# HKPolyU-UAV/FLVIS

Measured on AMD Instinct MI355X. Metric: frames/sec/node (640×480 stereo+IMU) + ATE vs CPU ref, EuRoC MH_05, higher is better.
Workload: dtype u8/f32 LK+GFTT, f64 geometry+BA

## Files before the change

### flvis_amd/csrc/dev_geom.hpp

```cpp
#pragma once
#include "dev_math.hpp"

namespace flvis {

FD void project_point(const float* p3, const M3& R, V3 t, const double* K, const double* D, float* out) {
  V3 P{(double)p3[0], (double)p3[1], (double)p3[2]};
  V3 X = R * P + t;
  double z = X.z ? 1. / X.z : 1;
  double x = X.x * z, y = X.y * z;
  double r2 = x * x + y * y, r4 = r2 * r2;
  double a1 = 2 * x * y, a2 = r2 + 2 * x * x, a3 = r2 + 2 * y * y;
  double cdist = 1 + D[0] * r2 + D[1] * r4;
  double xd = x * cdist + D[2] * a1 + D[3] * a2;
  double yd = y * cdist + D[2] * a3 + D[3] * a1;
  out[0] = (float)(xd * K[0] + K[2]);
  out[1] = (float)(yd * K[1] + K[3]);
}

FD void undistort_point(const float* src, const double* K, const double* D, const double* R9, const double* P12,
                        float* dst) {
  double x = (src[0] - K[2]) / K[0], y = (src[1] - K[3]) / K[1];
  double x0 = x, y0 = y;
  for (int j = 0; j < 5; j++) {
    double r2 = x * x + y * y;
    double icdist = 1. / (1 + (D[1] * r2 + D[0]) * r2);
    double deltaX = 2 * D[2] * x * y + D[3] * (r2 + 2 * x * x);
    double deltaY = D[2] * (r2 + 2 * y * y) + 2 * D[3] * x * y;
    x = (x0 - deltaX) * icdist;
    y = (y0 - deltaY) * icdist;
  }
  double xx = R9[0] * x + R9[1] * y + R9[2];
  double yy = R9[3] * x + R9[4] * y + R9[5];
  double ww = 1. / (R9[6] * x + R9[7] * y + R9[8]);
  x = xx * ww;
  y = yy * ww;
  dst[0] = (float)(x * P12[0] + P12[2]);
  dst[1] = (float)(y * P12[5] + P12[6]);
}

__device__ inline V3 triangulate_dlt(double u1, double v1, double u2, double v2, const double* P1, const double* P2) {
  double A[4][4], V[4][4];
#pragma unroll
  for (int j = 0; j < 4; j++) {
    A[0][j] = v1 * P1[8 + j] - P1[4 + j];
    A[1][j] = P1[j] - u1 * P1[8 + j];
    A[2][j] = v2 * P2[8 + j] - P2[4 + j];
    A[3][j] = P2[j] - u2 * P2[8 + j];
  }
#pragma unroll
  for (int i = 0; i < 4; i++)
#pragma unroll
    for (int j = 0; j < 4; j++) V[i][j] = (i == j) ? 1.0 : 0.0;
  for (int sweep = 0; sweep < 30; sweep++) {
    int off = 0;
#pragma unroll
    for (int p = 0; p < 3; p++)
#pragma unroll
      for (int q = p + 1; q < 4; q++) {
        double alpha = 0, beta = 0, gamma = 0;
#pragma unroll
        for (int i = 0; i < 4; i++) {
          alpha += A[i][p] * A[i][p];
          beta += A[i][q] * A[i][q];
          gamma += A[i][p] * A[i][q];
        }
        if (gamma * gamma <= 4.930380657631324e-30 * (alpha * beta)) continue;
        off = 1;
        double zeta = (beta - alpha) / (2.0 * gamma);
        double t = (zeta >= 0 ? 1.0 : -1.0) / (fabs(zeta) + sqrt(1.0 + zeta * zeta));
        double c = 1.0 / sqrt(1.0 + t * t), s = c * t;
#pragma unroll
        for (int i = 0; i < 4; i++) {
          double ap = A[i][p], aq = A[i][q];
          A[i][p] = c * ap - s * aq;
          A[i][q] = s * ap + c * aq;
          double vp = V[i][p], vq = V[i][q];
          V[i][p] = c * vp - s * vq;
          V[i][q] = s * vp + c * vq;
        }
      }
    if (!off) break;
  }
  int best = 0;
  double bn = 1.7976931348623157e308;
#pragma unroll
  for (int j = 0; j < 4; j++) {
    double nn = 0;
#pragma unroll
    for (int i = 0; i < 4; i++) nn += A[i][j] * A[i][j];
    if (nn < bn) {
      bn = nn;
      best = j;
    }
  }
  double vx = 0, vy = 0, vz = 0, vw = 1;
#pragma unroll
  for (int j = 0; j < 4; j++)
    if (j == best) {
      vx = V[0][j];
      vy = V[1][j];
      vz = V[2][j];
      vw = V[3][j];
    }
  return V3{vx / vw, vy / vw, vz / vw};
}

__device__ inline V3 triangulate_two_view(double u1, double v1, double u2, double v2, const SE3d& T1, const SE3d& T2,
                                          double fx, double fy, double cx, double cy) {
  double P1[12], P2[12];
  for (int k = 0; k < 2; k++) {
    const SE3d& T = k == 0 ? T1 : T2;
    double* P = k == 0 ? P1 : P2;
    M3 R = q_to_mat(T.q);
    double T34[3][4] = {{R.m[0][0], R.m[0][1], R.m[0][2], T.t.x}, {R.m[1][0], R.m[1][1], R.m[1][2], T.t.y},
                        {R.m[2][0], R.m[2][1], R.m[2][2], T.t.z}};
    for (int j = 0; j < 4; j++) {
      P[j] = fx * T34[0][j] + 0 * T34[1][j] + cx * T34[2][j];
      P[4 + j] = 0 * T34[0][j] + fy * T34[1][j] + cy * T34[2][j];
      P[8 + j] = 0 * T34[0][j] + 0 * T34[1][j] + 1 * T34[2][j];
    }
  }
  return triangulate_dlt(u1, v1, u2, v2, P1, P2);
}

FD float f_error(const double* F, double x1, double y1, double x2, double y2) {
  double a = F[0] * x1 + F[1] * y1 + F[2], b = F[3] * x1 + F[4] * y1 + F[5], c = F[6] * x1 + F[7] * y1 + F[8];
  double s2 = 1. / (a * a + b * b);
  double dd2 = x2 * a + y2 * b + c;
  a = F[0] * x2 + F[3] * y2 + F[6];
  b = F[1] * x2 + F[4] * y2 + F[7];
  c = F[2] * x2 + F[5] * y2 + F[8];
  double s1 = 1. / (a * a + b * b);
  double dd1 = x1 * a + y1 * b + c;
  return (float)fmax(dd1 * dd1 * s1, dd2 * dd2 * s2);
}

FD void proj_edge(const SE3d& T, V3 pw, double zu, double zv, double fx, double fy, double cx, double cy, double* e,
                  double (*J)[6]) {
  V3 X = g2o_map(T, pw);
  double x = X.x, y = X.y, zz = X.z, z2 = zz * zz;
  e[0] = zu - (x / zz * fx + cx);
  e[1] = zv - (y / zz * fy + cy);
  if (J) {
    J[0][0] = x * y / z2 * fx;
    J[0][1] = -(1 + (x * x / z2)) * fx;
    J[0][2] = y / zz * fx;
    J[0][3] = -1. / zz * fx;
    J[0][4] = 0;
    J[0][5] = x / z2 * fx;
    J[1][0] = (1 + y * y / z2) * fy;
    J[1][1] = -x * y / z2 * fy;
    J[1][2] = -x / zz * fy;
    J[1][3] = 0;
    J[1][4] = -1. / zz * fy;
    J[1][5] = y / z2 * fy;
// ... 36 lines not shown
```

### flvis_amd/csrc/frame_schedule.cpp

```cpp
#include <algorithm>
#include <chrono>
#include <cstring>
#include <thread>
#include <vector>

#include "pipeline_host.hpp"

using namespace flvis;

static void fill_pyr(Pipeline* pl, PyrSel& ps, uint8_t* const* l0, uint8_t* const* l1, const int* cur, int flip, int levels) {
  ps.levels = levels;
  for (int l = 0; l <= levels; l++) {
    ps.lvl[l] = ImgSel{{l0[l], l1 ? l1[l] : l0[l]}, cur, flip, nullptr};
    ps.w[l] = pl->lw[l];
    ps.h[l] = pl->lh[l];
    ps.pitch[l] = pl->lpitch[l];
    ps.stride[l] = pl->lstride[l];
    ps.bx[l] = pl->lbx;
    ps.by[l] = pl->lby;
  }
}

unsigned flvis::pyramid_levels(hipStream_t ds, bool bordered, ImgSel src0, int spitch0, size_t sstride0, bool ingest, bool level0_is_buffer,
                               const PyrSel& pyr, int S, const int* active) {
// ... 328 lines not shown
  {
    LaunchJoins j(pl, L, st, p.kj);
    head_signals = !pl->feedback_used && j.fold_signal(J_HEAD);
    head_posts = !idle_step && j.fold_post(J_IMG);
    if (head_prepare) launch_frame_head_prepare(st, p, L->d_time, L->d_progress, frame_no);
    else launch_frame_head(st, p, L->d_time, L->d_progress, frame_no);
  }
  if (pl->feedback_used) launch_apply_correction(st, p);
  pe(0, st);
  if (!head_signals) join_signal(pl, L, J_HEAD, st);
}

void Frame::local_map_tail(hipEvent_t* p18, bool timed) {
  if (with_local_map && (pl->frames_fed % pl->ba_every) == 0) {
    if (L->ba_pending) launch_local_map(pl, L, J_FE, true, nullptr);
    if (pl->defer_ba) L->ba_pending = true;
    else if (L->endf_valid) launch_local_map(pl, L, J_ENDF, false, p18);
    else launch_local_map(pl, L, J_FE, true, p18);
  } else if (!with_local_map) {
    if (cmd_pending) {
      if (L->ba_launches > 0) join_wait(pl, L, st, J_BA(L->ba_launches - 1));
      launch_kfq_drop(st, p);
    } else hipMemcpyAsync(p.kfq_head, p.kfq_tail, sizeof(unsigned) * S, hipMemcpyDeviceToDevice, st);
    if (timed) {
      pb(18, st);
      pe(18, st);
      L->prof18_rec[(size_t)pl->prof_step] = 1;
    }
  }
}

void Frame::frame_end(bool backpressure, bool with_innovate) {
  LaunchJoins j(pl, L, st, p.kj);
  if (with_innovate) j.wait(J_TRI);
  if (backpressure) lane_backpressure_wait(pl, L, &j, 0, with_innovate ? 1 : pl->nba_lane);
  pb(with_innovate ? 16 : 17, st);
  L->endf_valid = j.fold_signal(J_ENDF);
  if (with_innovate) launch_depth_innovate_end(st, p);
  else launch_frame_end(st, p);
  j.end();
  if (with_innovate) {
    pe(16, st);
    pb(17, st);
  }
  pe(17, st);
  pe(19, st);
}

void Frame::stage_idle_tail() {
  frame_end(false, false);
  if (prof)
    for (int i = 1; i < PROF_STAGES; i++)
      if (i != 17 && i != 19) {
        pb(i, st);
        pe(i, st);
      }
  if (!skipped) local_map_tail(nullptr, false);
}

LKParams Frame::lk_params(int stats_at, int tc_mode, int order) const {
  LKParams prm{30, 1e-3 * 1e-3, 1e-4f, 1};
  if (pl->lk_stats) prm.stats = reinterpret_cast<unsigned long long*>(p.counters) + stats_at;
  if (pl->lk_stats) prm.stats_tc = reinterpret_cast<unsigned long long*>(p.counters) + 61;
  if (L->tc) {
    prm.tc = L->tc;
    prm.tc_mode = tc_mode;
    prm.tc_cap = p.tc_cap;
// ... 58 lines not shown
  join_signal(pl, L, J_DET, ds);
}

void Frame::stage_pnp_pose() {
  pb(7, st);
  const bool ba_here = L->ba_pending;
  bool pnp_signals;
  {
    LaunchJoins j(pl, L, st, p.kj);
    pnp_signals = ba_here && j.fold_signal(J_FE);
    launch_ransac_pnp(st, p);
  }
  if (p.pnp_tail_cv) launch_pnp_tail_cv(st, p);
  pe(7, st);
  if (ba_here) launch_local_map(pl, L, J_FE, !pnp_signals, prof18);
  pb(8, st);
  if (merge_filter) {
    LaunchJoins j(pl, L, st, p.kj);
    j.signal(J_LM);
    launch_pose_lm_filter(st, p);
    pe(8, st);
    pb(9, st);
    pe(9, st);
  } else {
    launch_pose_lm(st, p);
    pe(8, st);
    pb(9, st);
    LaunchJoins j(pl, L, st, p.kj);
    j.signal(J_LM);
    launch_reproj_filter(st, p);
    pe(9, st);
  }
  join_wait(pl, L, ds, J_LM);
  launch_vi_correction(ds, p);
}

void Frame::stage_new_landmarks() {
  if (!merge_dem) {
    KJoin dem_kj{};
    LaunchJoins j(pl, L, st, dem_kj);
    j.wait(J_GFTT);
    pb(13, st);
    launch_feature_dem(st, w, h, S, p.cam.dem, L->dem_sorted, L->dem_roff, 2 * p.cam.gftt_num, p.det_mode, p.exist_xy, p.n_exist, NMAX,
                       p.new_xy, p.n_new, NEW_MAX, &dem_kj);
  }
  const bool merge_seeds = (pl->chain_merge & 1) != 0;
  const DemLaunch dem{w, h, L->dem_sorted, L->dem_roff, 2 * p.cam.gftt_num};
  bool an_signals, seeds_post;
  {
    LaunchJoins j(pl, L, st, p.kj);
    if (merge_dem) {
      j.wait(J_GFTT);
      pb(13, st);
    }
    if (merge_end && with_local_map) lane_backpressure_wait(pl, L, &j, 1, pl->nba_lane);
    an_signals = j.fold_signal(J_LM);
    if (!merge_seeds) {
      if (merge_dem) launch_dem_add_new_seeds(st, p, dem, false);
      else launch_add_new(st, p);
      j.end();
    }
    pe(13, st);
    pb(14, st);
    seeds_post = j.fold_post(J_DET);
    if (!merge_seeds) launch_depth_seeds(st, p);
    else if (merge_dem) launch_dem_add_new_seeds(st, p, dem, true);
    else launch_add_new_seeds(st, p);
  }
  pe(14, st);
  if (!an_signals) join_signal(pl, L, J_LM, st);
  join_wait(pl, L, ds, J_LM);
  launch_depth_triangulate(ds, p);
  join_signal(pl, L, J_TRI, ds);
  if (!seeds_post) join_wait(pl, L, st, J_DET);
}

void Frame::stage_stereo_depth() {
  pb(15, st);
  if (!depth_cam) {
    PyrSel prev, next;
    fill_pyr(pl, prev, L->pyr0[0], L->pyr0[1], p.img_slot, 0, pl->levels_s);
    fill_pyr(pl, next, L->pyr1, nullptr, nullptr, 0, pl->levels_s);
    next.lvl[0] = r_in_place ? in1 : img_plain(L->pyr1[0]);
    next.pitch[0] = r_in_place ? w : pl->lpitch[0];
    next.stride[0] = r_in_place ? (size_t)w * h : pl->lstride[0];
    if (r_in_place) next.bx[0] = next.by[0] = 0;
    launch_lk_track(st, prev, next, p.prev_pts, p.next_pts, p.lk_status, p.lk_count, NMAX, S, lk_params(48, 1, 1), p.det_mode, pl->max_pts, 2);
  }
  pe(15, st);
  if (merge_end) return;
  LaunchJoins j(pl, L, st, p.kj);
  j.wait(J_TRI);
  pb(16, st);
  launch_depth_innovate(st, p);
  j.end();
  pe(16, st);
}

void Frame::stage_frame_end() {
  frame_end(with_local_map != 0, merge_end);
  if (pl->kfl.cap > 0) kf_log_frame(pl, L, st, in1.b[0], depth_cam || r_in_place);
  local_map_tail(prof18, prof);
}

}

static void lane_frame(Pipeline* pl, Lane* L, const uint8_t* d_img0, const uint8_t* d_img1, const double* h_times, const uint8_t* present,
                       int with_local_map) {
  Frame f{pl, L, L->pipe, L->st, L->det_stream, L->S, pl->cfg.image_width, pl->cfg.image_height, with_local_map};
  f.stage_host_inputs(d_img0, d_img1, h_times, present);
  f.pb(19, f.st);
  if (!f.idle_step) f.stage_ingest_left();
  f.stage_head();
  if (f.idle_step) return f.stage_idle_tail();
  f.stage_temporal_lk();
  f.stage_collect_ransac_f();
  f.stage_detection_fork();
  f.stage_pnp_pose();
  f.stage_new_landmarks();
  f.stage_stereo_depth();
  f.stage_frame_end();
}

extern "C" {

// ... 96 lines not shown
```

### flvis_amd/csrc/pipeline.cpp

```cpp
#include <algorithm>
#include <chrono>
#include <cmath>
#include <cstddef>
#include <cstdio>
#include <cstdlib>
#include <cstring>
#include <thread>
#include <limits>
#include <vector>

#include "pipeline_host.hpp"

using namespace flvis;

static const char* kStageNames[PROF_STAGES] = {
    "imu_feed+frame_begin", "ingest(equalize)", "pyr_down(left)", "track_prepare", "lk_track(temporal)", "track_collect",
    "ransac_f", "ransac_pnp", "track_post+pose_lm", "reproj_filter", "gftt:eig_cand", "gftt:(merged)", "gftt:pick",
    "feature_dem+add_new", "depth_prepare", "lk_track(stereo)", "depth_innovate", "frame_end",
    "ba_worker(launch)", "frame(chain)"};

namespace {

int lk_levels(int w, int h, int win, int max_level) {
  int level = 0;
// ... 202 lines not shown
  CamParams& c = p.cam;
  c.cam_type = cfg->cam_type;
  c.w = w;
  c.h = h;
  c.need_equal_hist = cfg->need_equal_hist;
  c.skip_first_n = cfg->skip_first_n_imgs;
  c.dem.regionWidth = (int)std::floor(w / 4.0);
  c.dem.regionHeight = (int)std::floor(h / 4.0);
  c.dem.boundary_dis = (int)std::floor(cfg->feature_para[2] / 2.0);
  c.dem.max_region_feature_num = (unsigned)cfg->feature_para[0];
  c.gftt_num = (int)cfg->feature_para[3];
  c.gftt_ql = cfg->feature_para[4];
  c.gftt_dis = (int)cfg->feature_para[5];
  c.window = cfg->window_size;
  c.seed = seed_base;

  bool ok = true;
#define DA(field, T, n) ok = ok && ((p.field = dalloc<T>(L->allocs, (n))) != nullptr)
  RigParams* rig = dalloc<RigParams>(L->allocs, S);
  ok = ok && rig;
  p.rig = rig;
  DA(st, StreamState, S);
  DA(lm, Landmark, (size_t)2 * S * NMAX);
  DA(vi, MotionState, (size_t)S * VI_QUEUE);
  DA(imu_out, double, (size_t)S * IMU_OUT_CAP * 11);
  DA(prev_pts, float, (size_t)S * NMAX * 2);
  DA(next_pts, float, (size_t)S * NMAX * 2);
  DA(lk_status, uint8_t, (size_t)S * NMAX);
  DA(lk_count, int, S);
  DA(lk_slot, int, (size_t)S * NMAX);
  DA(lk_tag, long long, S);
  DA(m1, float, (size_t)S * NMAX * 2);
  DA(m2, float, (size_t)S * NMAX * 2);
  DA(tri, double, (size_t)S * NMAX * 3);
  DA(tri_mask, uint8_t, (size_t)S * NMAX);
  DA(new_xy, float, (size_t)S * NEW_MAX * 2);
  DA(n_new, int, S);
  DA(exist_xy, double, (size_t)S * NMAX * 2);
  DA(n_exist, int, S);
  DA(act_img, int, S);
  DA(act_track, int, S);
  DA(det_mode, int, S);
  DA(det_maxc, int, S);
  DA(gftt_act, int, S);
  DA(gftt_maxc, int, S);
  DA(img_slot, int, S);
  DA(img_slot_in, int, S);
  DA(out, FrameOut, S);
  DA(kfq, KeyFrameDev, (size_t)S * KFQ);
  DA(kfq_tail, unsigned, S);
  DA(kfq_head, unsigned, S);
  DA(kfq_cmd, unsigned, S);
  DA(kfq_skip, unsigned, S);
  DA(kfq_base, unsigned, S);
  DA(kfq_kf, unsigned, S);
  DA(ba_busy, int, S);
  DA(win, WindowDev, S);
  DA(kfs_ring, KeyFrameDev, (size_t)S * BA_WMAX);
  DA(corr, CorrectionDev, S);
  DA(rec_id, int, (size_t)S * POSE_REC);
  DA(rec_T, double, (size_t)S * POSE_REC * 7);
  p.corr_in = nullptr;
  DA(counters, long long, 64);
  p.ba_scratch_stride = ba_scratch_doubles();
  p.imu_factor = 0;
  p.imu_sigma_g = 0;
  p.imu_sigma_a = 0;
  p.ba_drain = 1;
// ... 1244 lines not shown
```

### flvis_amd/csrc/pipeline_host.hpp

```cpp
#pragma once
#include <vector>

#include "../../include/flvis_hip.h"
#include "ctx.hpp"
#include "kf_log.hpp"
#include "lm_cloud.hpp"
#include "track_kernels.hpp"

namespace flvis {

constexpr int PROF_STAGES = 20;

constexpr int BAQ = 64;
enum JoinId {
  J_IMG,
  J_DET,
  J_GFTT,
  J_FE,
  J_LM,
  J_TRI,
  J_HEAD,
  J_ENDF,
  J_BA0,
  JOIN_IDS = J_BA0 + BAQ
};
inline JoinId J_BA(long long launch) { return (JoinId)(J_BA0 + (int)(launch % BAQ)); }
struct Join {
  hipEvent_t ev = nullptr;
  long long* word = nullptr;
  unsigned* cnt = nullptr;
  long long seq = 0;
};

struct Lane {
  int s0 = 0, S = 0;
  Pipe pipe;
  hipStream_t st = nullptr;
  bool own_st = false;
  uint8_t* pyr0[2][LK_MAX_LEVELS] = {};
  uint8_t* pyr1[LK_MAX_LEVELS] = {};
  uint32_t* tc = nullptr;
  int tc_stride = 0;
  GfttScratch gftt;
  float* gftt_xy = nullptr;
  float* dem_sorted = nullptr;
  int* dem_roff = nullptr;
  int* gftt_n = nullptr;
  unsigned* eq_hist = nullptr;
  uint8_t* eq_lut = nullptr;
  uint8_t* d_inputs = nullptr;
  double* d_time = nullptr;
  const uint8_t** d_tab = nullptr;
  size_t input_bytes = 0;
// ... 137 lines not shown
```

### flvis_amd/csrc/track_kernels.hip

```cpp
#include <vector>

#include "dev_common.hpp"
#include "dev_geom.hpp"
#include "epnp_core.hpp"
#include "feature_dem_dev.hpp"
#include "track_kernels.hpp"
#include "cv_solvers.hpp"
#include "vi_motion.hpp"

namespace flvis {

FD Landmark* lm_ptr(const Pipe& p, int slot, int s) { return p.lm + ((size_t)slot * p.S + s) * NMAX; }

extern __shared__ __attribute__((aligned(16))) unsigned char pl_smem[];

FD int glibc_rand_next(StreamState& st) {
  int pos = st.rnd_pos;
  int a = st.rnd_r[(pos + 34 - 31) % 34], b = st.rnd_r[(pos + 34 - 3) % 34];
  int n = (int)((unsigned)a + (unsigned)b);
  st.rnd_r[pos] = n;
  st.rnd_pos = (pos + 1) % 34;
  return (int)(((unsigned)n) >> 1);
}

// ... 1947 lines not shown
    const int i = c * T + tid;
    const bool keep = i < n && !(d[c] > sh);
    Landmark lm;
    if (keep) lm = lms[i];
    int tot;
    const int k = kept + block_rank<T / 64>(keep, s_cnt, tot);
    if (keep) {
      lm.inlier = 1;
      lms[k] = lm;
      double* ex = p.exist_xy + ((size_t)s * NMAX + k) * 2;
      ex[0] = lm.p2d[0];
      ex[1] = lm.p2d[1];
    }
    kept += tot;
  }
  if (tid == 0) {
    st.n_lm[cur] = kept;
    st.orig_size = kept;
    p.n_exist[s] = kept;
    p.det_mode[s] = 2;
    p.det_maxc[s] = p.cam.gftt_num;
    st.vi_corr_due = st.has_imu ? 1 : 0;
  }
}
__global__ __launch_bounds__(PL_T) void k_pose_lm_filter(Pipe p) {
  kj_wait(p.kj);
  k_pose_lm_body(p);
  __syncthreads();
  reproj_filter_chunks_dev<PL_T>(p, reinterpret_cast<PoseLMShared*>(pl_smem)->terms);
  kj_signal(p.kj);
}
__global__ void k_vi_correction(Pipe p) {
  const int s = blockIdx.x * blockDim.x + threadIdx.x;
  if (s >= p.S) return;
  StreamState& st = p.st[s];
  if (!st.vi_corr_due) return;
  st.vi_corr_due = 0;
  const int cur = st.cur;
  ViRing ring{p.vi + (size_t)s * VI_QUEUE, &st};
  vi_correction_from_vision(rig_of(p, s), st, ring, st.frame_time[cur], load_pose7(st.T_c_w[cur]), st.frame_time[cur ^ 1],
                            load_pose7(st.T_c_w[cur ^ 1]));
}

template <int T>
__device__ __forceinline__ void k_add_new_body(const Pipe& p) {
  const int s = blockIdx.x;
  CRig& rg = rig_of(p, s);
  StreamState& st = p.st[s];
  const int mode = p.det_mode[s];
  if (mode == 0) return;
  const int lane = threadIdx.x;
  const int cur = st.cur;
  Landmark* lms = lm_ptr(p, cur, s);
  int n0 = st.n_lm[cur];
  int nn = p.n_new[s];
  if (n0 + nn > NMAX) nn = NMAX - n0;
  const float* xy = p.new_xy + (size_t)s * NEW_MAX * 2;
  const bool as_inlier = (mode == 1) ? true : (st.orig_size < 60);
  for (int k = lane; k < nn; k += T) {
    float src[2] = {xy[2 * k], xy[2 * k + 1]};
    float und[2] = {src[0], src[1]};
    if ((mode == 1 && p.cam.cam_type != CAM_DEPTH) || p.cam.cam_type == CAM_STEREO_UNRECT)
      undistort_point(src, rig_arr(rg.K0).v, rig_arr(rg.D0).v, rig_arr(rg.R0).v, rig_arr(rg.P0).v, und);
    Landmark lm;
    lm.id = st.lm_id_counter + k;
    lm.p3w[0] = lm.p3w[1] = lm.p3w[2] = 0;
    lm.p3c[0] = lm.p3c[1] = lm.p3c[2] = 0;
    lm.p2d[0] = (double)src[0];
    lm.p2d[1] = (double)src[1];
    lm.p2u[0] = (double)und[0];
    lm.p2u[1] = (double)und[1];
    lm.first2d[0] = lm.p2u[0];
    lm.first2d[1] = lm.p2u[1];
    for (int j = 0; j < 7; j++) lm.first_pose[j] = st.T_c_w[cur][j];
// ... 52 lines not shown
  kj_wait(p.kj);
  k_depth_seeds_body(p);
  kj_signal(p.kj);
  kj_post_wait(p.kj);
}
__global__ __launch_bounds__(256) void k_add_new_seeds(Pipe p) {
  kj_wait(p.kj);
  const int s = blockIdx.x;
  if (p.det_mode[s] != 0) {
    k_add_new_body<256>(p);
    __syncthreads();
    for (int i = threadIdx.x; i < NMAX; i += 256) depth_seed_dev(p, s, i);
  }
  kj_signal(p.kj);
  kj_post_wait(p.kj);
}
static_assert(DEM_T == 256, "k_dem_add_new_seeds: FeatureDEM's body, k_add_new_body<256> and the seeds share one workgroup");
__global__ __launch_bounds__(256) void k_dem_add_new_seeds(Pipe p, DemLaunch d, int with_seeds) {
  kj_wait(p.kj);
  const int s = blockIdx.x;
  k_feature_dem_body(d.w, d.h, p.cam.dem, d.sorted_xy, d.region_off, d.corner_cap, p.det_mode, p.exist_xy, p.n_exist, NMAX, p.new_xy, p.n_new,
                     NEW_MAX);
  __syncthreads();
  if (p.det_mode[s] != 0) {
    k_add_new_body<256>(p);
    if (with_seeds) {
      __syncthreads();
      for (int i = threadIdx.x; i < NMAX; i += 256) depth_seed_dev(p, s, i);
    }
  }
  kj_signal(p.kj);
  kj_post_wait(p.kj);
}
__device__ __forceinline__ void k_depth_triangulate_body(const Pipe& p) {
  const int s = blockIdx.y;
  CRig& rg = rig_of(p, s);
  const StreamState& st = p.st[s];
  if (p.det_mode[s] == 0) return;
  const int cur = st.cur;
  const int n = st.n_lm[cur];
  const int i = blockIdx.x * 256 + threadIdx.x;
  if (i >= n) return;
  const Landmark& lm = lm_ptr(p, cur, s)[i];
  const SE3d T = load_pose7(st.T_c_w[cur]);
  SE3d T1 = load_pose7(lm.first_pose);
  V3 baseline = T1.t - T.t;
  double* tri = p.tri + ((size_t)s * NMAX + i) * 3;
  unsigned char tm = 0;
  tri[0] = tri[1] = tri[2] = 0;
  if (norm(baseline) >= 0.2) {
    V3 pw = triangulate_two_view(lm.first2d[0], lm.first2d[1], lm.p2u[0], lm.p2u[1], T1, T, rg.fx, rg.fy, rg.cx,
                                 rg.cy);
    V3 pc = se3_act(T, pw);
    if (pc.z >= 0.5 && pc.z <= (double)rg.range) {
      tri[0] = pc.x;
      tri[1] = pc.y;
      tri[2] = pc.z;
      tm = 1;
    }
  }
  p.tri_mask[(size_t)s * NMAX + i] = tm;
}
__global__ __launch_bounds__(256) void k_depth_triangulate(Pipe p) {
  kj_wait(p.kj);
  k_depth_triangulate_body(p);
  kj_signal(p.kj);
}

__device__ __forceinline__ void k_depth_innovate_body(const Pipe& p) {
  const int s = blockIdx.x;
  CRig& rg = rig_of(p, s);
  StreamState& st = p.st[s];
  if (p.det_mode[s] == 0) return;
  const int i = threadIdx.x;
  const int cur = st.cur;
  Landmark* lms = lm_ptr(p, cur, s);
  const int n = st.n_lm[cur];
  __shared__ float rnd[NMAX];
  __shared__ int s_cnt[NMAX / 64];
  const float* p1 = p.next_pts + (size_t)s * NMAX * 2;
  const uint8_t* status = p.lk_status + (size_t)s * NMAX;
  const double range = (double)rg.range;
  const bool valid = i < n;
  Landmark lm;
  bool ok = false;
  V3 meas{0, 0, 0};
  const bool depth_cam = p.cam.cam_type == CAM_DEPTH;
  float ptx = 0.f, pty = 0.f;
  if (valid) {
    lm = lms[i];
    if (depth_cam) {
      ptx = (float)round(lm.p2d[0]);
      pty = (float)round(lm.p2d[1]);
      const int ix = min(max(__float2int_rn(ptx), 0), p.cam.w - 1), iy = min(max(__float2int_rn(pty), 0), p.cam.h - 1);
      const uint16_t d16 = reinterpret_cast<const uint16_t*>(p.in_img1)[(size_t)s * p.cam.w * p.cam.h + (size_t)iy * p.cam.w + ix];
      const float z = (float)((double)d16 / rg.depth_scale);
      if ((double)z >= 0.3 && z <= rg.range) {
        meas = V3{((double)ptx - rg.cx) * (double)z / rg.fx, ((double)pty - rg.cy) * (double)z / rg.fy, (double)z};
        ok = true;
      }
    } else if (status[i] == 1) {
      float src[2] = {p1[2 * i], p1[2 * i + 1]}, u1[2];
      undistort_point(src, rig_arr(rg.K1).v, rig_arr(rg.D1).v, rig_arr(rg.R1).v, rig_arr(rg.P1).v, u1);
      float u0x = (float)lm.p2u[0], u0y = (float)lm.p2u[1];
      V3 pc = triangulate_dlt((double)u0x, (double)u0y, (double)u1[0], (double)u1[1], rig_arr(rg.P0).v, rig_arr(rg.P1).v);
      if (!(pc.z < 0 || pc.z > range)) {
        meas = pc;
        ok = true;
      }
    }
  }
  int nfail;
  const int frank = block_rank<NMAX / 64>(valid && !ok, s_cnt, nfail);
  if (i == 0)
    for (int k = 0; k < nfail; k++)
      rnd[k] = (float)(0.3 + (double)((float)glibc_rand_next(st) / ((float)(2147483647 / (0.4)))));
  __syncthreads();
  if (valid) {
    const SE3d T = load_pose7(st.T_c_w[cur]);
    const SE3d Tinv = se3_inverse(T);
    const float iir = rg.iir_ratio;
    const bool tm = p.tri_mask[(size_t)s * NMAX + i] != 0;
    if (!ok) {
      double depth = (double)rnd[frank];
      if (depth_cam) {
        meas = V3{(lm.p2d[0] - rg.cx) * depth / rg.fx, (lm.p2d[1] - rg.cy) * depth / rg.fy, depth};
      } else {
        float u0x = (float)lm.p2u[0], u0y = (float)lm.p2u[1];
        meas = V3{((double)u0x - rg.cx) * depth / rg.fx, ((double)u0y - rg.cy) * depth / rg.fy, depth};
      }
    }
    if (!ok && !tm) {
      if (!depth_cam && !lm.has3d && rg.enable_dummy) {
        V3 pw = se3_act(Tinv, meas);
        lm.p3c[0] = meas.x; lm.p3c[1] = meas.y; lm.p3c[2] = meas.z;
        lm.p3w[0] = pw.x; lm.p3w[1] = pw.y; lm.p3w[2] = pw.z;
        lm.has3d = 1;
      }
    } else {
      V3 m = meas;
      if (!ok) {
        const double* tri = p.tri + ((size_t)s * NMAX + i) * 3;
        m = V3{tri[0], tri[1], tri[2]};
      }
      if (lm.has3d) {
        V3 lc = se3_act(T, V3{lm.p3w[0], lm.p3w[1], lm.p3w[2]});
        V3 upd = lc * (double)iir + m * (double)(1 - iir);
        V3 pw = se3_act(Tinv, upd);
        lm.p3c[0] = upd.x; lm.p3c[1] = upd.y; lm.p3c[2] = upd.z;
        lm.p3w[0] = pw.x; lm.p3w[1] = pw.y; lm.p3w[2] = pw.z;
      } else {
        V3 pw = se3_act(Tinv, m);
        lm.p3c[0] = m.x; lm.p3c[1] = m.y; lm.p3c[2] = m.z;
        lm.p3w[0] = pw.x; lm.p3w[1] = pw.y; lm.p3w[2] = pw.z;
        lm.has3d = 1;
      }
    }
  }
  int kept;
  const bool keep = valid && lm.has3d;
  const int k = block_rank<NMAX / 64>(keep, s_cnt, kept);
  if (keep) lms[k] = lm;
  if (i == 0) st.n_lm[cur] = kept;
}
__global__ __launch_bounds__(NMAX) void k_depth_innovate(Pipe p) {
  kj_wait(p.kj);
  k_depth_innovate_body(p);
  kj_signal(p.kj);
}

constexpr int FE_T = 256;
template <int T>
__device__ __forceinline__ void k_frame_end_body(const Pipe& p) {
  const int s = blockIdx.x;
  StreamState& st = p.st[s];
  const int lane = threadIdx.x;
  __shared__ int s_newkf;
// ... 386 lines not shown
    }
    e = hipMemcpyToSymbol(HIP_SYMBOL(g_f_sub7), s7.data(), s7.size() * sizeof(unsigned short));
    if (e == hipSuccess) e = hipMemcpyToSymbol(HIP_SYMBOL(g_f_rng7), r7.data(), r7.size() * sizeof(unsigned long long));
    if (e != hipSuccess) return e;
  }
  e = hipMemcpyToSymbol(HIP_SYMBOL(g_pnp_sub5), s5.data(), s5.size() * sizeof(unsigned short));
  if (e == hipSuccess) e = hipMemcpyToSymbol(HIP_SYMBOL(g_pnp_sub4), s4.data(), s4.size() * sizeof(unsigned short));
  if (e == hipSuccess) e = hipMemcpyToSymbol(HIP_SYMBOL(g_pnp_rng5), r5.data(), r5.size() * sizeof(unsigned long long));
  if (e == hipSuccess) e = hipMemcpyToSymbol(HIP_SYMBOL(g_pnp_rng4), r4.data(), r4.size() * sizeof(unsigned long long));
  if (e == hipSuccess && dev >= 0 && dev < 64) done[dev] = true;
  return e;
}
hipError_t track_kernels_init() {
  {
    const hipError_t e = pnp_tables_init();
    if (e != hipSuccess) return e;
  }
  {
    const hipError_t e = hipFuncSetAttribute((const void*)k_pose_lm_filter, hipFuncAttributeMaxDynamicSharedMemorySize, (int)sizeof(PoseLMShared));
    if (e != hipSuccess) return e;
  }
  return hipFuncSetAttribute((const void*)k_pose_lm, hipFuncAttributeMaxDynamicSharedMemorySize, (int)sizeof(PoseLMShared));
}
void launch_reproj_filter(hipStream_t st, const Pipe& p) { hipLaunchKernelGGL(k_reproj_filter, dim3(p.S), dim3(NMAX), 0, st, p); }
void launch_vi_correction(hipStream_t st, const Pipe& p) { hipLaunchKernelGGL(k_vi_correction, dim3((p.S + 63) / 64), dim3(64), 0, st, p); }
void launch_add_new(hipStream_t st, const Pipe& p) { hipLaunchKernelGGL(k_add_new, dim3(p.S), dim3(64), 0, st, p); }
void launch_depth_seeds(hipStream_t st, const Pipe& p) {
  hipLaunchKernelGGL(k_depth_seeds, dim3(NMAX / 256, p.S), dim3(256), 0, st, p);
}
void launch_add_new_seeds(hipStream_t st, const Pipe& p) { hipLaunchKernelGGL(k_add_new_seeds, dim3(p.S), dim3(256), 0, st, p); }
void launch_dem_add_new_seeds(hipStream_t st, const Pipe& p, const DemLaunch& d, bool with_seeds) {
  hipLaunchKernelGGL(k_dem_add_new_seeds, dim3(p.S), dim3(256), dem_body_lds(d.corner_cap), st, p, d, with_seeds ? 1 : 0);
}
void launch_depth_triangulate(hipStream_t st, const Pipe& p) {
  hipLaunchKernelGGL(k_depth_triangulate, dim3(NMAX / 256, p.S), dim3(256), 0, st, p);
}
void launch_depth_innovate(hipStream_t st, const Pipe& p) { hipLaunchKernelGGL(k_depth_innovate, dim3(p.S), dim3(NMAX), 0, st, p); }
void launch_frame_end(hipStream_t st, const Pipe& p) {
  hipLaunchKernelGGL(k_frame_end, dim3(p.S), dim3(FE_T), 0, st, p);
}
void launch_depth_innovate_end(hipStream_t st, const Pipe& p) {
  hipLaunchKernelGGL(k_depth_innovate_end, dim3(p.S), dim3(NMAX), 0, st, p);
}

}
```

### flvis_amd/csrc/track_kernels.hpp

```cpp
#pragma once
#include "pipeline.hpp"

namespace flvis {

constexpr int NEW_MAX = 1024;

struct Pipe {
  int S;
  CamParams cam;
  const RigParams* rig;
  StreamState* st;
  Landmark* lm;
  MotionState* vi;
  const unsigned long long* seeds;
  double* imu_in;
  int* n_imu;
  const int* present;
  double* imu_out;
  float* prev_pts;
  float* next_pts;
  uint8_t* lk_status;
  int* lk_count;
  int* lk_slot;
  long long* lk_tag;
  int tc_cap;
  const uint32_t* tc;
  int tc_stride;
  float* m1;
  float* m2;
  double* tri;
  uint8_t* tri_mask;
  float* new_xy;
  int* n_new;
  double* exist_xy;
  int* n_exist;
  int* act_img;
  int* act_track;
  int* det_mode;
  int* det_maxc;
  int* gftt_act;
  int* gftt_maxc;
  int* img_slot;
  int* img_slot_in;
  FrameOut* out;
  double* traj;
  int traj_cap;
  KeyFrameDev* kfq;
  unsigned* kfq_tail;
  unsigned* kfq_head;
  unsigned* kfq_cmd;
  unsigned* kfq_skip;
  unsigned* kfq_base;
  unsigned* kfq_kf;
  int* ba_busy;
  WindowDev* win;
  KeyFrameDev* kfs_ring;
  CorrectionDev* corr;
  double* ba_scratch;
  size_t ba_scratch_stride;
  int imu_factor;
  double imu_sigma_a;
  double imu_sigma_g;
  int ba_lds_bytes;
  int ba_drain;
// ... 44 lines not shown
hipError_t launch_pose_lm_sets(hipStream_t st, const double* lm3d, const double* lm2d, const long long* lm_id, const int* count, int cap,
                               int n_sets, const double* d_K4, int k_stride, double* pose7, unsigned char* ok);
constexpr int GEOM_CAM_N = 29;
void launch_undistort_points_sets(hipStream_t st, const float* src, const int* count, int cap, int n_sets, const double* d_cam, int cam_stride,
                                  float* dst);
void launch_project_points_sets(hipStream_t st, const float* p3d, const int* count, int cap, int n_sets, const double* d_pose7,
                                const double* d_cam, int cam_stride, float* dst);
void launch_store_progress(hipStream_t st, long long* host_word, long long v);
void launch_store_flag(hipStream_t st, long long* word, long long v);
void launch_wait_flag(hipStream_t st, const long long* flag, int n_words, long long seq, long long* err_word);
void launch_frame_head(hipStream_t st, const Pipe& p, const double* d_time, long long* host_progress, long long frame_no);
void launch_frame_head_prepare(hipStream_t st, const Pipe& p, const double* d_time, long long* host_progress, long long frame_no);
void launch_apply_correction(hipStream_t st, const Pipe& p);
void launch_track_prepare(hipStream_t st, const Pipe& p);
void launch_track_collect(hipStream_t st, const Pipe& p);
void launch_ransac_f(hipStream_t st, const Pipe& p, bool with_collect = false);
void launch_ransac_pnp(hipStream_t st, const Pipe& p);
void launch_pnp_tail_cv(hipStream_t st, const Pipe& p);
void launch_track_post(hipStream_t st, const Pipe& p);
void launch_pose_lm(hipStream_t st, const Pipe& p);
void launch_reproj_filter(hipStream_t st, const Pipe& p);
void launch_pose_lm_filter(hipStream_t st, const Pipe& p);
void launch_vi_correction(hipStream_t st, const Pipe& p);
void launch_add_new(hipStream_t st, const Pipe& p);
void launch_depth_seeds(hipStream_t st, const Pipe& p);
void launch_add_new_seeds(hipStream_t st, const Pipe& p);
struct DemLaunch {
  int w, h;
  const float* sorted_xy;
  const int* region_off;
  int corner_cap;
};
void launch_dem_add_new_seeds(hipStream_t st, const Pipe& p, const DemLaunch& d, bool with_seeds);
void launch_depth_triangulate(hipStream_t st, const Pipe& p);
void launch_depth_innovate(hipStream_t st, const Pipe& p);
void launch_frame_end(hipStream_t st, const Pipe& p);
void launch_depth_innovate_end(hipStream_t st, const Pipe& p);
constexpr int RESET_LIST = 64;
enum { RS_TRACKER = 1, RS_CMD = 2, RS_SKIP = 4, RS_CREATE = 8 };
struct ResetList {
  int n;
  int s[RESET_LIST];
  unsigned char mode[RESET_LIST];
};
void launch_stream_reset(hipStream_t st, const Pipe& p, const ResetList& list, long long* err_word);
void launch_kfq_drop(hipStream_t st, const Pipe& p);
void launch_set_rig(hipStream_t st, const Pipe& p, int ls, const RigParams& r);
void launch_ba_worker(hipStream_t st, const Pipe& p);
hipError_t ba_kernels_init();
hipError_t track_kernels_init();
size_t ba_scratch_doubles();

}
```

Before: 63160.

## Fuse two-view depth triangulation into depth-innovate kernel and drop tri buffers

Removes the separate k_depth_triangulate kernel and its global tri/tri_mask scratch buffers. The two-view DLT is now computed inside k_depth_innovate, sharing one Jacobi SVD call with the stereo path per thread, plus a wave-uniform fallback pass for stereo points rejected by range. The join that used to follow triangulation now keys on vi_correction, which signals at its end. This saves a kernel launch, a cross-stream join and global round trips, at the cost of more register pressure and divergence in the innovate kernel. Two-view triangulation is now only computed for landmarks without a valid stereo measurement.

Measured after the change: 63360 (median of 5 runs). No clear change (+0.3%).

```diff
diff --git a/flvis_amd/csrc/dev_geom.hpp b/flvis_amd/csrc/dev_geom.hpp
--- a/flvis_amd/csrc/dev_geom.hpp
+++ b/flvis_amd/csrc/dev_geom.hpp
@@ -38,15 +38,15 @@
   dst[1] = (float)(y * P12[5] + P12[6]);
 }
 
-__device__ inline V3 triangulate_dlt(double u1, double v1, double u2, double v2, const double* P1, const double* P2) {
-  double A[4][4], V[4][4];
+FD void dlt_rows(double u, double v, const double* P, double* row_v, double* row_u) {
 #pragma unroll
   for (int j = 0; j < 4; j++) {
-    A[0][j] = v1 * P1[8 + j] - P1[4 + j];
-    A[1][j] = P1[j] - u1 * P1[8 + j];
-    A[2][j] = v2 * P2[8 + j] - P2[4 + j];
-    A[3][j] = P2[j] - u2 * P2[8 + j];
-  }
+    row_v[j] = v * P[8 + j] - P[4 + j];
+    row_u[j] = P[j] - u * P[8 + j];
+  }
+}
+__device__ inline V3 dlt_null_vector(double (&A)[4][4]) {
+  double V[4][4];
 #pragma unroll
   for (int i = 0; i < 4; i++)
 #pragma unroll
@@ -104,23 +104,40 @@
     }
   return V3{vx / vw, vy / vw, vz / vw};
 }
-
+__device__ inline V3 triangulate_dlt(double u1, double v1, double u2, double v2, const double* P1, const double* P2) {
+  double A[4][4];
+  dlt_rows(u1, v1, P1, A[0], A[1]);
+  dlt_rows(u2, v2, P2, A[2], A[3]);
+  return dlt_null_vector(A);
+}
+
+__device__ inline void dlt_rows_pose(double u, double v, const SE3d& T, double fx, double fy, double cx, double cy, double* row_v,
+                                     double* row_u) {
+  double P[12];
+  M3 R = q_to_mat(T.q);
+  double T34[3][4] = {{R.m[0][0], R.m[0][1], R.m[0][2], T.t.x}, {R.m[1][0], R.m[1][1], R.m[1][2], T.t.y},
+                      {R.m[2][0], R.m[2][1], R.m[2][2], T.t.z}};
+#pragma unroll
+  for (int j = 0; j < 4; j++) {
+    P[j] = fx * T34[0][j] + 0 * T34[1][j] + cx * T34[2][j];
+    P[4 + j] = 0 * T34[0][j] + fy * T34[1][j] + cy * T34[2][j];
+    P[8 + j] = 0 * T34[0][j] + 0 * T34[1][j] + 1 * T34[2][j];
+  }
+  dlt_rows(u, v, P, row_v, row_u);
+}
+__device__ inline void dlt_rows_two_view(double u1, double v1, double u2, double v2, const SE3d& T1, const SE3d& T2, double fx, double fy,
+                                         double cx, double cy, double (&A)[4][4]) {
+  dlt_rows_pose(u1, v1, T1, fx, fy, cx, cy, A[0], A[1]);
+#if defined(__HIP_DEVICE_COMPILE__)
+  __builtin_amdgcn_sched_barrier(0);
+#endif
+  dlt_rows_pose(u2, v2, T2, fx, fy, cx, cy, A[2], A[3]);
+}
 __device__ inline V3 triangulate_two_view(double u1, double v1, double u2, double v2, const SE3d& T1, const SE3d& T2,
                                           double fx, double fy, double cx, double cy) {
-  double P1[12], P2[12];
-  for (int k = 0; k < 2; k++) {
-    const SE3d& T = k == 0 ? T1 : T2;
-    double* P = k == 0 ? P1 : P2;
-    M3 R = q_to_mat(T.q);
-    double T34[3][4] = {{R.m[0][0], R.m[0][1], R.m[0][2], T.t.x}, {R.m[1][0], R.m[1][1], R.m[1][2], T.t.y},
-                        {R.m[2][0], R.m[2][1], R.m[2][2], T.t.z}};
-    for (int j = 0; j < 4; j++) {
-      P[j] = fx * T34[0][j] + 0 * T34[1][j] + cx * T34[2][j];
-      P[4 + j] = 0 * T34[0][j] + fy * T34[1][j] + cy * T34[2][j];
-      P[8 + j] = 0 * T34[0][j] + 0 * T34[1][j] + 1 * T34[2][j];
-    }
-  }
-  return triangulate_dlt(u1, v1, u2, v2, P1, P2);
+  double A[4][4];
+  dlt_rows_two_view(u1, v1, u2, v2, T1, T2, fx, fy, cx, cy, A);
+  return dlt_null_vector(A);
 }
 
 FD float f_error(const double* F, double x1, double y1, double x2, double y2) {
diff --git a/flvis_amd/csrc/frame_schedule.cpp b/flvis_amd/csrc/frame_schedule.cpp
--- a/flvis_amd/csrc/frame_schedule.cpp
+++ b/flvis_amd/csrc/frame_schedule.cpp
@@ -384,7 +384,7 @@
 
 void Frame::frame_end(bool backpressure, bool with_innovate) {
   LaunchJoins j(pl, L, st, p.kj);
-  if (with_innovate) j.wait(J_TRI);
+  if (with_innovate) j.wait(J_VIC);
   if (backpressure) lane_backpressure_wait(pl, L, &j, 0, with_innovate ? 1 : pl->nba_lane);
   pb(with_innovate ? 16 : 17, st);
   L->endf_valid = j.fold_signal(J_ENDF);
@@ -509,6 +509,8 @@
     pe(9, st);
   }
   join_wait(pl, L, ds, J_LM);
+  LaunchJoins j(pl, L, ds, p.kj);
+  j.signal(J_VIC);
   launch_vi_correction(ds, p);
 }
 
@@ -523,7 +525,7 @@
   }
   const bool merge_seeds = (pl->chain_merge & 1) != 0;
   const DemLaunch dem{w, h, L->dem_sorted, L->dem_roff, 2 * p.cam.gftt_num};
-  bool an_signals, seeds_post;
+  bool seeds_post;
   {
     LaunchJoins j(pl, L, st, p.kj);
     if (merge_dem) {
@@ -531,7 +533,6 @@
       pb(13, st);
     }
     if (merge_end && with_local_map) lane_backpressure_wait(pl, L, &j, 1, pl->nba_lane);
-    an_signals = j.fold_signal(J_LM);
     if (!merge_seeds) {
       if (merge_dem) launch_dem_add_new_seeds(st, p, dem, false);
       else launch_add_new(st, p);
@@ -545,10 +546,6 @@
     else launch_add_new_seeds(st, p);
   }
   pe(14, st);
-  if (!an_signals) join_signal(pl, L, J_LM, st);
-  join_wait(pl, L, ds, J_LM);
-  launch_depth_triangulate(ds, p);
-  join_signal(pl, L, J_TRI, ds);
   if (!seeds_post) join_wait(pl, L, st, J_DET);
 }
 
@@ -567,7 +564,7 @@
   pe(15, st);
   if (merge_end) return;
   LaunchJoins j(pl, L, st, p.kj);
-  j.wait(J_TRI);
+  j.wait(J_VIC);
   pb(16, st);
   launch_depth_innovate(st, p);
   j.end();
diff --git a/flvis_amd/csrc/pipeline.cpp b/flvis_amd/csrc/pipeline.cpp
--- a/flvis_amd/csrc/pipeline.cpp
+++ b/flvis_amd/csrc/pipeline.cpp
@@ -258,8 +258,6 @@
   DA(lk_tag, long long, S);
   DA(m1, float, (size_t)S * NMAX * 2);
   DA(m2, float, (size_t)S * NMAX * 2);
-  DA(tri, double, (size_t)S * NMAX * 3);
-  DA(tri_mask, uint8_t, (size_t)S * NMAX);
   DA(new_xy, float, (size_t)S * NEW_MAX * 2);
   DA(n_new, int, S);
   DA(exist_xy, double, (size_t)S * NMAX * 2);
diff --git a/flvis_amd/csrc/pipeline_host.hpp b/flvis_amd/csrc/pipeline_host.hpp
--- a/flvis_amd/csrc/pipeline_host.hpp
+++ b/flvis_amd/csrc/pipeline_host.hpp
@@ -18,7 +18,7 @@
   J_GFTT,
   J_FE,
   J_LM,
-  J_TRI,
+  J_VIC,
   J_HEAD,
   J_ENDF,
   J_BA0,
diff --git a/flvis_amd/csrc/track_kernels.hip b/flvis_amd/csrc/track_kernels.hip
--- a/flvis_amd/csrc/track_kernels.hip
+++ b/flvis_amd/csrc/track_kernels.hip
@@ -2003,14 +2003,15 @@
 }
 __global__ void k_vi_correction(Pipe p) {
   const int s = blockIdx.x * blockDim.x + threadIdx.x;
-  if (s >= p.S) return;
-  StreamState& st = p.st[s];
-  if (!st.vi_corr_due) return;
-  st.vi_corr_due = 0;
-  const int cur = st.cur;
-  ViRing ring{p.vi + (size_t)s * VI_QUEUE, &st};
-  vi_correction_from_vision(rig_of(p, s), st, ring, st.frame_time[cur], load_pose7(st.T_c_w[cur]), st.frame_time[cur ^ 1],
-                            load_pose7(st.T_c_w[cur ^ 1]));
+  if (s < p.S && p.st[s].vi_corr_due) {
+    StreamState& st = p.st[s];
+    st.vi_corr_due = 0;
+    const int cur = st.cur;
+    ViRing ring{p.vi + (size_t)s * VI_QUEUE, &st};
+    vi_correction_from_vision(rig_of(p, s), st, ring, st.frame_time[cur], load_pose7(st.T_c_w[cur]), st.frame_time[cur ^ 1],
+                              load_pose7(st.T_c_w[cur ^ 1]));
+  }
+  kj_signal(p.kj);
 }
 
 template <int T>
@@ -2129,41 +2130,20 @@
   kj_signal(p.kj);
   kj_post_wait(p.kj);
 }
-__device__ __forceinline__ void k_depth_triangulate_body(const Pipe& p) {
-  const int s = blockIdx.y;
-  CRig& rg = rig_of(p, s);
-  const StreamState& st = p.st[s];
-  if (p.det_mode[s] == 0) return;
-  const int cur = st.cur;
-  const int n = st.n_lm[cur];
-  const int i = blockIdx.x * 256 + threadIdx.x;
-  if (i >= n) return;
-  const Landmark& lm = lm_ptr(p, cur, s)[i];
-  const SE3d T = load_pose7(st.T_c_w[cur]);
-  SE3d T1 = load_pose7(lm.first_pose);
+
+FD bool two_view_rows(const Landmark& lm, const SE3d& T, CRig& rg, double (&A)[4][4]) {
+  const SE3d T1 = load_pose7(lm.first_pose);
   V3 baseline = T1.t - T.t;
-  double* tri = p.tri + ((size_t)s * NMAX + i) * 3;
-  unsigned char tm = 0;
-  tri[0] = tri[1] = tri[2] = 0;
-  if (norm(baseline) >= 0.2) {
-    V3 pw = triangulate_two_view(lm.first2d[0], lm.first2d[1], lm.p2u[0], lm.p2u[1], T1, T, rg.fx, rg.fy, rg.cx,
-                                 rg.cy);
-    V3 pc = se3_act(T, pw);
-    if (pc.z >= 0.5 && pc.z <= (double)rg.range) {
-      tri[0] = pc.x;
-      tri[1] = pc.y;
-      tri[2] = pc.z;
-      tm = 1;
-    }
-  }
-  p.tri_mask[(size_t)s * NMAX + i] = tm;
-}
-__global__ __launch_bounds__(256) void k_depth_triangulate(Pipe p) {
-  kj_wait(p.kj);
-  k_depth_triangulate_body(p);
-  kj_signal(p.kj);
-}
-
+  if (!(norm(baseline) >= 0.2)) return false;
+  dlt_rows_two_view(lm.first2d[0], lm.first2d[1], lm.p2u[0], lm.p2u[1], T1, T, rg.fx, rg.fy, rg.cx, rg.cy, A);
+  return true;
+}
+FD bool two_view_accept(V3 pw, const SE3d& T, double range, V3& tri) {
+  const V3 pc = se3_act(T, pw);
+  if (!(pc.z >= 0.5 && pc.z <= range)) return false;
+  tri = pc;
+  return true;
+}
 __device__ __forceinline__ void k_depth_innovate_body(const Pipe& p) {
   const int s = blockIdx.x;
   CRig& rg = rig_of(p, s);
@@ -2184,11 +2164,13 @@
   V3 meas{0, 0, 0};
   const bool depth_cam = p.cam.cam_type == CAM_DEPTH;
   float ptx = 0.f, pty = 0.f;
+  double A[4][4];
+  bool stereo = false, two_view = false, tm = false;
   if (valid) {
-    lm = lms[i];
+    const Landmark& g = lms[i];
     if (depth_cam) {
-      ptx = (float)round(lm.p2d[0]);
-      pty = (float)round(lm.p2d[1]);
+      ptx = (float)round(g.p2d[0]);
+      pty = (float)round(g.p2d[1]);
       const int ix = min(max(__float2int_rn(ptx), 0), p.cam.w - 1), iy = min(max(__float2int_rn(pty), 0), p.cam.h - 1);
       const uint16_t d16 = reinterpret_cast<const uint16_t*>(p.in_img1)[(size_t)s * p.cam.w * p.cam.h + (size_t)iy * p.cam.w + ix];
       const float z = (float)((double)d16 / rg.depth_scale);
@@ -2199,13 +2181,26 @@
     } else if (status[i] == 1) {
       float src[2] = {p1[2 * i], p1[2 * i + 1]}, u1[2];
       undistort_point(src, rig_arr(rg.K1).v, rig_arr(rg.D1).v, rig_arr(rg.R1).v, rig_arr(rg.P1).v, u1);
-      float u0x = (float)lm.p2u[0], u0y = (float)lm.p2u[1];
-      V3 pc = triangulate_dlt((double)u0x, (double)u0y, (double)u1[0], (double)u1[1], rig_arr(rg.P0).v, rig_arr(rg.P1).v);
-      if (!(pc.z < 0 || pc.z > range)) {
-        meas = pc;
-        ok = true;
-      }
-    }
+      float u0x = (float)g.p2u[0], u0y = (float)g.p2u[1];
+      dlt_rows((double)u0x, (double)u0y, rig_arr(rg.P0).v, A[0], A[1]);
+      dlt_rows((double)u1[0], (double)u1[1], rig_arr(rg.P1).v, A[2], A[3]);
+      stereo = true;
+    }
+    if (!ok && !stereo) two_view = two_view_rows(g, load_pose7(st.T_c_w[cur]), rg, A);
+  }
+  if (stereo || two_view) {
+    const V3 x = dlt_null_vector(A);
+    if (two_view) {
+      tm = two_view_accept(x, load_pose7(st.T_c_w[cur]), range, meas);
+    } else if (!(x.z < 0 || x.z > range)) {
+      meas = x;
+      ok = true;
+    }
+  }
+  const bool again = stereo && !ok;
+  if (__ballot(again) != 0ull) {
+    if (again && two_view_rows(lms[i], load_pose7(st.T_c_w[cur]), rg, A))
+      tm = two_view_accept(dlt_null_vector(A), load_pose7(st.T_c_w[cur]), range, meas);
   }
   int nfail;
   const int frank = block_rank<NMAX / 64>(valid && !ok, s_cnt, nfail);
@@ -2214,11 +2209,11 @@
       rnd[k] = (float)(0.3 + (double)((float)glibc_rand_next(st) / ((float)(2147483647 / (0.4)))));
   __syncthreads();
   if (valid) {
+    lm = lms[i];
     const SE3d T = load_pose7(st.T_c_w[cur]);
     const SE3d Tinv = se3_inverse(T);
     const float iir = rg.iir_ratio;
-    const bool tm = p.tri_mask[(size_t)s * NMAX + i] != 0;
-    if (!ok) {
+    if (!ok && !tm) {
       double depth = (double)rnd[frank];
       if (depth_cam) {
         meas = V3{(lm.p2d[0] - rg.cx) * depth / rg.fx, (lm.p2d[1] - rg.cy) * depth / rg.fy, depth};
@@ -2235,11 +2230,7 @@
         lm.has3d = 1;
       }
     } else {
-      V3 m = meas;
-      if (!ok) {
-        const double* tri = p.tri + ((size_t)s * NMAX + i) * 3;
-        m = V3{tri[0], tri[1], tri[2]};
-      }
+      const V3 m = meas;
       if (lm.has3d) {
         V3 lc = se3_act(T, V3{lm.p3w[0], lm.p3w[1], lm.p3w[2]});
         V3 upd = lc * (double)iir + m * (double)(1 - iir);
@@ -2692,9 +2683,6 @@
 void launch_dem_add_new_seeds(hipStream_t st, const Pipe& p, const DemLaunch& d, bool with_seeds) {
   hipLaunchKernelGGL(k_dem_add_new_seeds, dim3(p.S), dim3(256), dem_body_lds(d.corner_cap), st, p, d, with_seeds ? 1 : 0);
 }
-void launch_depth_triangulate(hipStream_t st, const Pipe& p) {
-  hipLaunchKernelGGL(k_depth_triangulate, dim3(NMAX / 256, p.S), dim3(256), 0, st, p);
-}
 void launch_depth_innovate(hipStream_t st, const Pipe& p) { hipLaunchKernelGGL(k_depth_innovate, dim3(p.S), dim3(NMAX), 0, st, p); }
 void launch_frame_end(hipStream_t st, const Pipe& p) {
   hipLaunchKernelGGL(k_frame_end, dim3(p.S), dim3(FE_T), 0, st, p);
diff --git a/flvis_amd/csrc/track_kernels.hpp b/flvis_amd/csrc/track_kernels.hpp
--- a/flvis_amd/csrc/track_kernels.hpp
+++ b/flvis_amd/csrc/track_kernels.hpp
@@ -28,8 +28,6 @@
   int tc_stride;
   float* m1;
   float* m2;
-  double* tri;
-  uint8_t* tri_mask;
   float* new_xy;
   int* n_new;
   double* exist_xy;
@@ -140,7 +138,6 @@
   int corner_cap;
 };
 void launch_dem_add_new_seeds(hipStream_t st, const Pipe& p, const DemLaunch& d, bool with_seeds);
-void launch_depth_triangulate(hipStream_t st, const Pipe& p);
 void launch_depth_innovate(hipStream_t st, const Pipe& p);
 void launch_frame_end(hipStream_t st, const Pipe& p);
 void launch_depth_innovate_end(hipStream_t st, const Pipe& p);
```
